# jaesung-cs/vulkan_radix_sort

Hardware: AMD Instinct MI355X
Metric: GItems/s at N=2^25 (keys & key+value); achieved HBM GB/s vs peak (higher is better)
Workload: dtype u32

## Files before the change

vulkan_radix_sort_amd/csrc/vrdx_kernels.hip:

```cpp
#include <hip/hip_runtime.h>
#include <stdint.h>

#include <type_traits>

#include "vrdx_kernels.h"
#include "vrdx_layout.h"

namespace vrdx {



#ifdef VRDX_TRACE
#define VRDX_STAMP(slot)                                      \
  do {                                                        \
    if (a.trace != nullptr && tid == 0) stamps[slot] = wall_clock64(); \
  } while (0)
#else
#define VRDX_STAMP(slot) \
  do {                   \
  } while (0)
#endif


typedef uint32_t u32x4 __attribute__((ext_vector_type(4)));
// ... 2120 lines not shown
    lo += v[k] & 0xFFFFu;
    hi += v[k] >> 16;
  }
  if (tid < 64u) {
    const uint32_t mine = tid < 2 * WORDS ? total[tid] : 0u;
    const uint32_t inclusive = WaveInclusiveScan(mine);
    if (tid < 2 * WORDS) {
      uint32_t base = inclusive - mine;
#pragma unroll
      for (uint32_t q = 0; q < 16; ++q) base += below[q];
      a.bucketBase[firstBucket + tid] = base;
      if (topWindow) a.bucketCount[firstBucket + tid] = mine;
      if (mine > a.cap) atomicOr(a.overflowWord, kMsdDeclineBucket);
    }
  }
}

template <uint32_t BITS, bool KV>
__device__ __forceinline__ void ScatterMsdBody(const MsdArgs a) {
  constexpr int THREADS = 1024, KPT = 32, WAVES = THREADS / 64;
  constexpr uint32_t TILE = kMsdTileKeys, D = 1u << BITS, ROW = D / 2u;
  static_assert(THREADS * KPT == TILE && ROW <= (uint32_t)THREADS && WAVES * ROW <= TILE, "geometry");
  extern __shared__ __attribute__((aligned(16))) uint32_t smem[];
  uint32_t* const sorted = smem;
  uint32_t* const counters = smem;
  uint32_t* const tileOffset = smem + TILE;
  uint32_t* const scanScratch = tileOffset + D;

  const int tid = threadIdx.x;
  const int lane = tid & 63;
  const int wave = tid >> 6;
  const uint32_t n = ElementCount(a.maxCount, a.countPtr);
  const uint32_t perXcd = gridDim.x / 8u;
  const uint32_t tile = (blockIdx.x % 8u) * perXcd + blockIdx.x / 8u;
  const uint32_t slots = a.tileKeys / (uint32_t)THREADS;
  const uint32_t frame = a.tileKeys;
  const uint32_t tileStart = tile * frame;
  const uint32_t decided = *a.overflowWord;
  if ((decided & kMsdDeclineMask) != 0u) {
    if (blockIdx.x == 0 && tid == 0 && a.declinedPlans != nullptr) atomicAdd(a.declinedPlans, 1u);
    return;
  }
  const uint32_t SHIFT = (decided >> kMsdShiftShift) & kMsdShiftMask;
  if (((decided >> kMsdModeShift) & kMsdModeMask) == kMsdModeIdentical) {
    if (blockIdx.x == 0 && tid == 0) *a.planWord = kMsdVerdictSorted;
    return;
  }
  const uint32_t valid = tile < a.tiles && tileStart < n ? ((n - tileStart) < frame ? (n - tileStart) : frame) : 0u;
  const uint32_t tileEnd = tileStart + valid;
  const uint32_t loadBase = tileStart + wave * (slots * 64) + lane;
  uint32_t key[KPT];
  LoadStriped<KPT, true, true>(a.keysCaller, loadBase, tileEnd, valid == frame, 0xFFFFFFFFu, key, slots);
  uint32_t prefixWord = 0, base0 = 0, base1 = 0;
  if ((uint32_t)tid < ROW && valid != 0) {
    prefixWord = a.tileCounts[(size_t)tile * ROW + tid];
    base0 = a.bucketBase[2 * tid];
    base1 = a.bucketBase[2 * tid + 1];
  }
  if (blockIdx.x == 0 && tid == 0) *a.planWord = kMsdVerdictRuns | (SHIFT << kMsdShiftShift);
  if (valid == 0) return;

  uint32_t* const myRow = counters + wave * ROW;
#pragma unroll
  for (uint32_t i = 0; i < ROW / 256u; ++i) reinterpret_cast<u32x4*>(myRow)[lane + 64 * i] = u32x4{0u, 0u, 0u, 0u};
  uint32_t rank[KPT / 2];
  RankPacked16<KPT, true>(key, SHIFT, BITS, myRow, lane, rank, slots);
  ForgetDerivedValues<KPT>(key);
  LdsBarrier();

  uint32_t column[WAVES];
  const uint32_t totals = (uint32_t)tid < ROW ? ColumnRead<ROW, WAVES>(counters, tid, column) : 0u;
  const uint32_t count0 = totals & 0xFFFFu, count1 = totals >> 16;
  const uint32_t local0 = BlockExclusiveScanAll<THREADS>(count0 + count1, scanScratch, tid);
  const uint32_t local1 = local0 + count0;
  if ((uint32_t)tid < ROW) {
    ColumnBasesFrom<ROW, WAVES>(counters, tid, local0 | (local1 << 16), column);
    tileOffset[2 * tid] = base0 + (prefixWord & 0xFFFFu) - local0;
    tileOffset[2 * tid + 1] = base1 + (prefixWord >> 16) - local1;
  }
  LdsBarrier();
  PositionsPacked16<KPT, TILE, true>(key, SHIFT, BITS, myRow, rank, slots);
  LdsBarrier();
#pragma unroll
  for (int i = 0; i < KPT; ++i) {
    if (i % 4 == 0 && (uint32_t)i >= slots) break;
    sorted[(rank[i / 2] >> (16 * (i % 2))) & 0xFFFFu] = key[i];
  }
  LdsBarrier();
  uint32_t val[KV ? KPT : 1];
  if constexpr (KV)
    LoadStriped<KPT, true, true>(a.valuesCaller, loadBase, tileEnd, valid == frame, 0u, val, slots);

  constexpr int QUADS = KPT / 4;
  constexpr int B = 4;
  uint32_t quadDigits[KV ? QUADS : 1];
  uint32_t boundaryQuad[2] = {~0u, ~0u};
  uint32_t boundaryDigits[2][2] = {{0, 0}, {0, 0}};
  if ((uint32_t)tid < ROW) {
    if (count0 != 0 && (local0 & 3u) != 0 && local0 < valid) boundaryQuad[0] = local0 & ~3u;
    if (count1 != 0 && (local1 & 3u) != 0 && local1 < valid) boundaryQuad[1] = local1 & ~3u;
  }
  if (tid == 0 && (valid & 3u) != 0) boundaryQuad[0] = valid & ~3u;
  auto scatterQuads = [&](uint32_t* out, bool keysPhase) {
#pragma unroll
    for (int j0 = 0; j0 < QUADS; j0 += B) {
      if (4u * (uint32_t)j0 * THREADS >= valid) break;
      u32x4 w4[B];
      uint32_t o[B];
      bool whole[B];
#pragma unroll
      for (int b = 0; b < B; ++b) w4[b] = *reinterpret_cast<const u32x4*>(&sorted[4u * (tid + (j0 + b) * THREADS)]);
#pragma unroll
      for (int b = 0; b < B; ++b) {
        const int j = j0 + b;
        const uint32_t p = StagingSlot<TILE>(4u * (tid + j * THREADS));
        uint32_t d0, d3;
        if (keysPhase) {
          d0 = __builtin_amdgcn_ubfe(w4[b][0], SHIFT, BITS);
          d3 = __builtin_amdgcn_ubfe(w4[b][3], SHIFT, BITS);
          if constexpr (KV) quadDigits[j] = d0 | (d3 << 16);
        } else {
          d0 = quadDigits[KV ? j : 0] & 0xFFFFu;
          d3 = quadDigits[KV ? j : 0] >> 16;
        }
        whole[b] = p + 3 < valid && d0 == d3;
        o[b] = tileOffset[d0] + p;
        asm volatile("" : "+v"(o[b]));
      }
#pragma unroll
      for (int b = 0; b < B; ++b)
        if (whole[b]) StoreQuad(out, o[b], w4[b]);
    }
#pragma unroll
    for (int s = 0; s < 2; ++s) {
      if (boundaryQuad[s] == ~0u) continue;
      const u32x4 q = *reinterpret_cast<const u32x4*>(&sorted[StagingSlot<TILE>(boundaryQuad[s])]);
      if (keysPhase) {
        boundaryDigits[s][0] = __builtin_amdgcn_ubfe(q[0], SHIFT, BITS) | (__builtin_amdgcn_ubfe(q[1], SHIFT, BITS) << 16);
        boundaryDigits[s][1] = __builtin_amdgcn_ubfe(q[2], SHIFT, BITS) | (__builtin_amdgcn_ubfe(q[3], SHIFT, BITS) << 16);
      }
#pragma unroll
      for (int c = 0; c < 4; ++c) {
        const uint32_t d = (boundaryDigits[s][c / 2] >> (16 * (c % 2))) & 0xFFFFu;
        if (boundaryQuad[s] + c < valid) StoreWord(out, tileOffset[d] + boundaryQuad[s] + c, q[c]);
      }
    }
  };
  scatterQuads(a.keysScratch, true);
  if constexpr (KV) {
    LdsBarrier();
#pragma unroll
    for (int i = 0; i < KPT; ++i) {
      if (i % 4 == 0 && (uint32_t)i >= slots) break;
      sorted[(rank[i / 2] >> (16 * (i % 2))) & 0xFFFFu] = val[i];
    }
    LdsBarrier();
    scatterQuads(a.valuesScratch, false);
  }
}

template <uint32_t BITS>
__device__ __forceinline__ void ScatterMsdPairBody(const MsdArgs a) {
  constexpr int THREADS = 1024, KPT = 32, WAVES = THREADS / 64;
  constexpr uint32_t TILE = kMsdTileKeys, D = 1u << BITS, ROW = D / 2u;
  static_assert(2 * WAVES * ROW <= TILE, "both sub-tiles' counter rows inside the staging buffer");
  extern __shared__ __attribute__((aligned(16))) uint32_t smem[];
  uint32_t* const sorted = smem;
  uint32_t* const counters = smem;
  uint32_t* const tileOffset = smem + TILE;
  uint32_t* const scanScratch = tileOffset + D;

  const int tid = threadIdx.x;
  const int lane = tid & 63;
  const int wave = tid >> 6;
  const uint32_t n = ElementCount(a.maxCount, a.countPtr);
  const uint32_t pairs = (a.tiles + 1u) / 2u;
  const uint32_t perXcd = (pairs + 7u) / 8u;
  const uint32_t pair = (blockIdx.x % 8u) * perXcd + blockIdx.x / 8u;
  const uint32_t slots = a.tileKeys / (uint32_t)THREADS;
  const uint32_t frame = a.tileKeys;
  const uint32_t decided = *a.overflowWord;
  if ((decided & kMsdDeclineMask) != 0u) {
    if (blockIdx.x == 0 && tid == 0 && a.declinedPlans != nullptr) atomicAdd(a.declinedPlans, 1u);
    return;
  }
  const uint32_t SHIFT = (decided >> kMsdShiftShift) & kMsdShiftMask;
  if (((decided >> kMsdModeShift) & kMsdModeMask) == kMsdModeIdentical) {
    if (blockIdx.x == 0 && tid == 0) *a.planWord = kMsdVerdictSorted;
    return;
  }
  const uint32_t tileA = 2u * pair;
  const uint32_t startA = tileA * frame, startB = startA + frame;
  const bool exists = blockIdx.x < 8u * perXcd && pair < pairs && startA < n;
  const uint32_t left = exists ? n - startA : 0u;
  const uint32_t validA = left < frame ? left : frame;
  const uint32_t validB = left > frame ? (left - frame < frame ? left - frame : frame) : 0u;
  const uint32_t valid = validA + validB;
  const uint32_t baseA = startA + wave * (slots * 64) + lane, baseB = baseA + frame;
  uint32_t keyA[KPT], keyB[KPT];
  LoadStriped<KPT, true, true>(a.keysCaller, baseA, startA + validA, validA == frame, 0xFFFFFFFFu, keyA, slots);
  LoadStriped<KPT, true, true>(a.keysCaller, baseB, startB + validB, validB == frame, 0xFFFFFFFFu, keyB, slots);
  uint32_t prefixWord = 0, base0 = 0, base1 = 0;
  if ((uint32_t)tid < ROW && valid != 0) {
    prefixWord = a.tileCounts[(size_t)tileA * ROW + tid];
    base0 = a.bucketBase[2 * tid];
    base1 = a.bucketBase[2 * tid + 1];
  }
  if (blockIdx.x == 0 && tid == 0) *a.planWord = kMsdVerdictRuns | (SHIFT << kMsdShiftShift);
  if (valid == 0) return;

  uint32_t* const rowA = counters + wave * ROW;
  uint32_t* const rowB = counters + (WAVES + wave) * ROW;
#pragma unroll
  for (uint32_t i = 0; i < ROW / 256u; ++i) {
    reinterpret_cast<u32x4*>(rowA)[lane + 64 * i] = u32x4{0u, 0u, 0u, 0u};
    reinterpret_cast<u32x4*>(rowB)[lane + 64 * i] = u32x4{0u, 0u, 0u, 0u};
  }
  uint32_t posA[KPT / 2], posB[KPT / 2];
  RankPacked16<KPT, true>(keyA, SHIFT, BITS, rowA, lane, posA, slots);
  ForgetDerivedValues<KPT>(keyA);
  RankPacked16<KPT, true>(keyB, SHIFT, BITS, rowB, lane, posB, slots);
  ForgetDerivedValues<KPT>(keyB);
  LdsBarrier();

  const uint32_t totals = (uint32_t)tid < ROW ? ColumnTotals<ROW, 2 * WAVES>(counters, tid) : 0u;
  const uint32_t count0 = totals & 0xFFFFu, count1 = totals >> 16;
  const uint32_t local0 = BlockExclusiveScanAll<THREADS>(count0 + count1, scanScratch, tid);
  const uint32_t local1 = local0 + count0;
  if ((uint32_t)tid < ROW) {
    ColumnBases<ROW, 2 * WAVES>(counters, tid, local0 | (local1 << 16));
    tileOffset[2 * tid] = base0 + (prefixWord & 0xFFFFu) - local0;
    tileOffset[2 * tid + 1] = base1 + (prefixWord >> 16) - local1;
  }
  LdsBarrier();
  PositionsPacked16<KPT, TILE, true, true>(keyA, SHIFT, BITS, rowA, posA, slots);
  PositionsPacked16<KPT, TILE, true, true>(keyB, SHIFT, BITS, rowB, posB, slots);
  LdsBarrier();

  constexpr int QUADS = KPT / 4;
  constexpr int B = 2;
  uint32_t boundaryQuad[2] = {~0u, ~0u};
  if ((uint32_t)tid < ROW) {
    if (count0 != 0 && (local0 & 3u) != 0 && local0 < valid) boundaryQuad[0] = local0 & ~3u;
    if (count1 != 0 && (local1 & 3u) != 0 && local1 < valid) boundaryQuad[1] = local1 & ~3u;
  }
  if (tid == 0 && (valid & 3u) != 0) boundaryQuad[0] = valid & ~3u;
#pragma unroll 1
  for (uint32_t half = 0; half < 2; ++half) {
    const uint32_t from = half * frame;
    if (from >= valid) break;
    if (half != 0) LdsBarrier();
#pragma unroll
    for (int i = 0; i < KPT; ++i) {
      if (i % 4 == 0 && (uint32_t)i >= slots) break;
      const uint32_t pa = ((posA[i / 2] >> (16 * (i % 2))) & 0xFFFFu) - from;
      const uint32_t pb = ((posB[i / 2] >> (16 * (i % 2))) & 0xFFFFu) - from;
      if (pa < frame) sorted[StagingSlot<TILE>(pa)] = keyA[i];
      if (pb < frame) sorted[StagingSlot<TILE>(pb)] = keyB[i];
    }
    LdsBarrier();
    const uint32_t here = valid - from < frame ? valid - from : frame;
#pragma unroll
    for (int j0 = 0; j0 < QUADS; j0 += B) {
      if (4u * (uint32_t)j0 * THREADS >= here) break;
      u32x4 w4[B];
      uint32_t o[B];
      bool whole[B];
#pragma unroll
      for (int b = 0; b < B; ++b) w4[b] = *reinterpret_cast<const u32x4*>(&sorted[4u * (tid + (j0 + b) * THREADS)]);
#pragma unroll
      for (int b = 0; b < B; ++b) {
        const uint32_t p = StagingSlot<TILE>(4u * (tid + (j0 + b) * THREADS));
        const uint32_t d0 = __builtin_amdgcn_ubfe(w4[b][0], SHIFT, BITS), d3 = __builtin_amdgcn_ubfe(w4[b][3], SHIFT, BITS);
        whole[b] = p + 3 < here && d0 == d3;
        o[b] = tileOffset[d0] + from + p;
        asm volatile("" : "+v"(o[b]));
      }
#pragma unroll
      for (int b = 0; b < B; ++b)
        if (whole[b]) StoreQuad(a.keysScratch, o[b], w4[b]);
    }
#pragma unroll
    for (int s = 0; s < 2; ++s) {
      const uint32_t q0 = boundaryQuad[s] - from;
      if (boundaryQuad[s] == ~0u || q0 >= frame) continue;
      const u32x4 q = *reinterpret_cast<const u32x4*>(&sorted[StagingSlot<TILE>(q0)]);
#pragma unroll
      for (int c = 0; c < 4; ++c)
        if (q0 + c < here) StoreWord(a.keysScratch, tileOffset[__builtin_amdgcn_ubfe(q[c], SHIFT, BITS)] + boundaryQuad[s] + c, q[c]);
    }
  }
}
template <uint32_t BITS, bool KV>
constexpr bool MsdScatterTakesPairs() { return !KV && BITS == 10; }
template <uint32_t BITS, bool KV>
__device__ __forceinline__ void ScatterMsdRole(const MsdArgs a) {
  if constexpr (MsdScatterTakesPairs<BITS, KV>())
    ScatterMsdPairBody<BITS>(a);
  else
    ScatterMsdBody<BITS, KV>(a);
}


template <uint32_t BITS, int KPT, bool KV, int THREADS = 1024>
__device__ __forceinline__ void BucketSort2Bucket(const MsdArgs a, const uint32_t bucket, const uint32_t below, const bool streamOut) {
  constexpr int WAVES = THREADS / 64;
  static_assert(THREADS == 1024 || THREADS == 512, "one or two words of a counter row per thread");
  constexpr uint32_t TILE = THREADS * KPT;
  constexpr uint32_t ROW = 1024;
  static_assert(32u - BITS <= 22u, "two passes of at most eleven bits");
  static_assert(TILE <= 65536 && WAVES * ROW <= TILE && KPT % 4 == 0, "packed positions; the staging buffer covers the counters");
  extern __shared__ __attribute__((aligned(16))) uint32_t smem[];
  uint32_t* const staged = smem;
  uint32_t* const counters = smem;
  uint32_t* const scanScratch = smem + TILE;

  const int tid = threadIdx.x;
  const int lane = tid & 63;
  const int wave = tid >> 6;
  const uint32_t W0 = (below + 1u) / 2u, W1 = below / 2u;
  constexpr uint32_t passes = 2u;
  const uint32_t myBase = (uint32_t)__builtin_amdgcn_readfirstlane((int)a.bucketBase[bucket]);
  const uint32_t n = (uint32_t)__builtin_amdgcn_readfirstlane((int)a.bucketCount[bucket]);
  if (n == 0) return;
  const uint32_t* const keysIn = a.keysScratch + myBase;
  uint32_t* const keysOut = a.keysCaller + myBase;
  const uint32_t* const valuesIn = KV ? a.valuesScratch + myBase : nullptr;
  uint32_t* const valuesOut = KV ? a.valuesCaller + myBase : nullptr;

  constexpr bool DYN = true;
  const uint32_t chunks = (n + 255u) / 256u;
  const uint32_t base = chunks / WAVES, extra = chunks % WAVES;
  const uint32_t w = (uint32_t)__builtin_amdgcn_readfirstlane(wave);
  const uint32_t slots = 4u * (base + (w < extra ? 1u : 0u));
  const uint32_t first = 256u * (w * base + (w < extra ? w : extra)) + lane;
  uint32_t key[KPT];
  uint32_t val[KV ? KPT : 1];
  LoadStriped<KPT, false, DYN>(keysIn, first, n, false, 0xFFFFFFFFu, key, slots);
  if constexpr (KV) LoadStriped<KPT, false, DYN>(valuesIn, first, n, false, 0u, val, slots);

  uint32_t* const myRow = counters + wave * ROW;
#pragma unroll 1
  for (uint32_t pass = 0; pass < passes; ++pass) {
    const uint32_t shift = pass == 0 ? 0u : W0;
    const uint32_t width = pass == 0 ? W0 : W1;
    const uint32_t words = width > 1u ? 1u << (width - 1u) : 1u;
#pragma unroll
    for (uint32_t i = 0; i < ROW / 256u; ++i)
      if (256u * i < words) reinterpret_cast<u32x4*>(myRow)[lane + 64 * i] = u32x4{0u, 0u, 0u, 0u};
    uint32_t rank[KPT / 2];
    RankPacked16<KPT, DYN>(key, shift, width, myRow, lane, rank, slots);
    ForgetDerivedValues<KPT>(key);
    LdsBarrier();
    uint32_t firstNow = first;
    asm volatile("" : "+v"(firstNow));
    if constexpr (THREADS == 512) {
      const bool mine = KV || 2u * (uint32_t)tid < words;
      u32x2 column[WAVES];
      const u32x2 totals = mine ? ColumnPairRead<ROW, WAVES>(counters, tid, column) : u32x2{0u, 0u};
      const uint32_t count0 = totals[0] & 0xFFFFu, count1 = totals[0] >> 16, count2 = totals[1] & 0xFFFFu;
      const uint32_t local0 = BlockExclusiveScanAll<THREADS>(count0 + count1 + count2 + (totals[1] >> 16), scanScratch + 16 * pass, tid);
      const uint32_t local2 = local0 + count0 + count1;
      if (mine)
        ColumnPairBasesFrom<ROW, WAVES>(counters, tid, u32x2{local0 | ((local0 + count0) << 16), local2 | ((local2 + count2) << 16)}, column);
    } else if constexpr (!KV) {
      const bool mine = (uint32_t)tid < words;
      uint32_t column[WAVES];
      const uint32_t totals = mine ? ColumnRead<ROW, WAVES>(counters, tid, column) : 0u;
      const uint32_t count0 = totals & 0xFFFFu;
      const uint32_t local0 = BlockExclusiveScanAll<THREADS>(count0 + (totals >> 16), scanScratch + 16 * pass, tid);
      if (mine) ColumnBasesFrom<ROW, WAVES>(counters, tid, local0 | ((local0 + count0) << 16), column);
    } else {
      const bool mine = (uint32_t)tid < words;
      const uint32_t totals = mine ? ColumnTotals<ROW, WAVES>(counters, tid) : 0u;
      const uint32_t count0 = totals & 0xFFFFu;
      const uint32_t local0 = BlockExclusiveScanAll<THREADS>(count0 + (totals >> 16), scanScratch + 16 * pass, tid);
      if (mine) ColumnBases<ROW, WAVES>(counters, tid, local0 | ((local0 + count0) << 16));
    }
    LdsBarrier();
    PositionsPacked16<KPT, TILE, DYN>(key, shift, width, myRow, rank, slots);
    LdsBarrier();
#pragma unroll
    for (int i = 0; i < KPT; ++i) {
      if (DYN && i % 4 == 0 && (uint32_t)i >= slots) break;
      staged[(rank[i / 2] >> (16 * (i % 2))) & 0xFFFFu] = key[i];
    }
    LdsBarrier();
#pragma unroll
    for (int i = 0; i < KPT; ++i) {
      if (DYN && i % 4 == 0 && (uint32_t)i >= slots) break;
      key[i] = staged[StagingSlot<TILE>(firstNow + 64 * i)];
    }
    if constexpr (KV) {
      LdsBarrier();
#pragma unroll
      for (int i = 0; i < KPT; ++i) {
        if (DYN && i % 4 == 0 && (uint32_t)i >= slots) break;
        staged[(rank[i / 2] >> (16 * (i % 2))) & 0xFFFFu] = val[i];
      }
      LdsBarrier();
#pragma unroll
      for (int i = 0; i < KPT; ++i) {
        if (DYN && i % 4 == 0 && (uint32_t)i >= slots) break;
        val[i] = staged[StagingSlot<TILE>(firstNow + 64 * i)];
      }
    }
    LdsBarrier();
  }
  if (KV ? a.maxCount > kStreamingLoadsAbove : streamOut) {
    asm volatile("; non-temporal output" ::: "memory");
#pragma unroll
    for (int i = 0; i < KPT; ++i) {
      if (DYN && i % 4 == 0 && (uint32_t)i >= slots) break;
      const uint32_t index = first + 64 * i;
      if (index < n) {
        __builtin_nontemporal_store(key[i], &keysOut[index]);
        if constexpr (KV) __builtin_nontemporal_store(val[i], &valuesOut[index]);
      }
    }
    asm volatile("" ::: "memory");
  } else {
#pragma unroll
    for (int i = 0; i < KPT; ++i) {
      if (DYN && i % 4 == 0 && (uint32_t)i >= slots) break;
      const uint32_t index = first + 64 * i;
      if (index < n) {
        keysOut[index] = key[i];
        if constexpr (KV) valuesOut[index] = val[i];
      }
    }
  }
}

template <uint32_t BITS, int KPT, bool KV, int THREADS = 1024>
__device__ __forceinline__ void BucketSort2Body(const MsdArgs a, const uint32_t workgroups) {
  const uint32_t verdict = *a.planWord;
  if ((verdict & kMsdVerdictMask) != kMsdVerdictRuns) return;
  const uint32_t below = (verdict >> kMsdShiftShift) & kMsdShiftMask;
  uint32_t streamedBuckets = 0u;
  if constexpr (!KV && THREADS == 1024 && BITS == 10)
    if (a.maxCount > kStreamingLoadsAbove) streamedBuckets = (1u << BITS) - min(a.plainTail, 1u << BITS);
#pragma unroll 1
  for (uint32_t bucket = blockIdx.x; bucket < (1u << BITS); bucket += workgroups)
    BucketSort2Bucket<BITS, KPT, KV, THREADS>(a, bucket, below, bucket < streamedBuckets);
}

template <uint32_t BITS, bool KV>
__global__ __launch_bounds__(512, 4) void bucket_sort2_half_kernel(MsdArgs a) {
  BucketSort2Body<BITS, kMsdHalfCap / 512, KV, 512>(a, gridDim.x);
}

template <uint32_t BITS, bool KV, bool DYN>
__device__ __forceinline__ void FallbackPassBody(const OnesweepArgs p) {
  if constexpr (KV)
    OnesweepBody<1024, 32, true, true, DYN>(p);
  else
    OnesweepPairBody<1024, 32, DYN>(p);
}

template <uint32_t BITS, bool KV, bool DYN>
__global__ __launch_bounds__(1024) void msd_scatter_or_pass0_kernel(MsdArgs m, OnesweepArgs p) {
  if ((*m.overflowWord & kMsdDeclineMask) == 0u) {
    ScatterMsdRole<BITS, KV>(m);
    return;
  }
  if (blockIdx.x > p.statusRows) return;
  FallbackPassBody<BITS, KV, DYN>(p);
  if (blockIdx.x == 0 && threadIdx.x == 0 && m.declinedPlans != nullptr) atomicAdd(m.declinedPlans, 1u);
}
template <uint32_t BITS, bool KV, bool DYN>
__global__ __launch_bounds__(1024) void msd_buckets_or_pass1_kernel(MsdArgs m, OnesweepArgs p) {
  const uint32_t verdict = *m.planWord & kMsdVerdictMask;
  if (verdict < kMsdVerdictRuns) {
    if (blockIdx.x > p.statusRows) return;
    FallbackPassBody<BITS, KV, DYN>(p);
    return;
  }
  const uint32_t workgroups = min(gridDim.x, (1u << BITS) / 2u);
  if (verdict == kMsdVerdictRuns && blockIdx.x < workgroups)
    BucketSort2Body<BITS, (KV ? kMsdCapKeyValue : kMsdCapKeys) / 1024, KV>(m, workgroups);
}

__device__ __forceinline__ uint32_t OrderCheckKey(uint32_t tid, uint32_t wave, uint32_t slot) {
  uint32_t x = (blockIdx.x * 1024u + tid) * 0x9E3779B9u + slot * 0x85EBCA6Bu;
  x ^= x >> 15; x *= 0x2C1B3C6Du; x ^= x >> 12; x *= 0x297A2D39u; x ^= x >> 15;
  const uint32_t mode = (blockIdx.x + wave + slot) % 6u;
  const uint32_t mask = mode == 0 ? 0u : mode == 1 ? 1u : mode == 2 ? 3u : mode == 3 ? 15u : mode == 4 ? 0x21u : 255u;
  return x & mask;
}

__global__ __launch_bounds__(1024) void lds_order_check_kernel(uint32_t* mismatches, uint32_t* sticky) {
  __shared__ uint32_t counters[2 * 16 * 256];
  const int tid = threadIdx.x, lane = tid & 63, wave = tid >> 6;
  for (int i = tid; i < 2 * 16 * 256; i += 1024) counters[i] = 0;
  __syncthreads();
  uint32_t* const histA = counters + wave * 256;
  uint32_t* const histB = counters + (16 + wave) * 256;
  uint32_t bad = 0;
  for (uint32_t round = 0; round < 8; ++round) {
    uint32_t key[8], ra[8], rb[8];
#pragma unroll
    for (int i = 0; i < 8; ++i) key[i] = OrderCheckKey(tid, wave, round * 8 + i);
    RankAtomic<8, false>(key, 0, histA, lane, ra);
    RankBallot<8>(key, 0, histB, lane, rb);
#pragma unroll
    for (int i = 0; i < 8; ++i) bad += ra[i] != rb[i];
  }
#pragma unroll 1
  for (uint32_t form = 0; form < 2; ++form) {
    uint32_t key[32], want[16];
#pragma unroll
    for (int i = 0; i < 32; ++i) key[i] = OrderCheckKey(tid, wave, 64 + 32 * form + i);
    RankBallot<32, true>(key, 0, histB, lane, want);
    if (form == 0) {
      uint32_t ra[32];
      RankAtomic<32, false>(key, 0, histA, lane, ra);
#pragma unroll
      for (int i = 0; i < 16; ++i) bad += (ra[2 * i] | (ra[2 * i + 1] << 16)) != want[i];
    } else {
      uint32_t rp[16];
      RankAtomic<32, true>(key, 0, histA, lane, rp);
#pragma unroll
      for (int i = 0; i < 16; ++i) bad += rp[i] != want[i];
    }
  }
  if (bad != 0) {
    if (mismatches != nullptr) atomicAdd(mismatches, bad);
    if (sticky != nullptr) atomicOr(sticky, 2u);
  }
}

__device__ __forceinline__ uint32_t OrderCheckDigit11(uint32_t tid, uint32_t wave, uint32_t slot) {
  uint32_t x = (blockIdx.x * 1024u + tid) * 0x9E3779B9u + slot * 0x85EBCA6Bu + 0x7F4A7C15u;
  x ^= x >> 15; x *= 0x2C1B3C6Du; x ^= x >> 12; x *= 0x297A2D39u; x ^= x >> 15;
  const uint32_t mode = (blockIdx.x + wave + slot) % 7u;
  const uint32_t mask = mode == 0 ? 0u : mode == 1 ? 1u : mode == 2 ? 3u : mode == 3 ? 15u : mode == 4 ? 0x421u : mode == 5 ? 63u : 2047u;
  return ((x & mask) + (mode == 5 ? 0x300u : 0u)) & 2047u;
}

__global__ __launch_bounds__(1024) void lds_order_check_packed_kernel(uint32_t* mismatches, uint32_t* sticky) {
  extern __shared__ __attribute__((aligned(16))) uint32_t smem[];
  const int tid = threadIdx.x, lane = tid & 63, wave = tid >> 6;
  uint32_t* const rowA = smem + wave * 1024;
  uint32_t* const rowB = smem + (16 + wave) * 1024;
  for (int i = lane; i < 1024; i += 64) rowA[i] = rowB[i] = 0;
  uint32_t bad = 0;
#pragma unroll 1
  for (uint32_t round = 0; round < 4; ++round) {
    uint32_t key[16], got[8];
#pragma unroll
    for (int i = 0; i < 16; ++i) key[i] = OrderCheckDigit11(tid, wave, round * 16 + i);
    RankPacked16<16, false>(key, 0, 11u, rowA, lane, got);
#pragma unroll
    for (int i = 0; i < 16; ++i) {
      const uint32_t d = key[i];
      uint64_t same = ~0ull;
#pragma unroll
      for (int b = 0; b < 11; ++b) {
        const bool bit = (d >> b) & 1u;
        const uint64_t ballot = __ballot(bit);
        same &= bit ? ballot : ~ballot;
      }
      const uint32_t below = LanesBelow(same);
      const uint32_t sh = (d & 1u) * 16u;
      const uint32_t prior = (__hip_atomic_load(&rowB[d >> 1], __ATOMIC_RELAXED, __HIP_MEMORY_SCOPE_WORKGROUP) >> sh) & 0xFFFFu;
      if (below == 0)
        (void)__hip_atomic_fetch_add(&rowB[d >> 1], (uint32_t)__popcll(same) << sh, __ATOMIC_RELAXED, __HIP_MEMORY_SCOPE_WORKGROUP);
      bad += ((got[i / 2] >> (16 * (i % 2))) & 0xFFFFu) != prior + below;
    }
  }
  if (bad != 0) {
    if (mismatches != nullptr) atomicAdd(mismatches, bad);
    if (sticky != nullptr) atomicOr(sticky, 2u);
  }
}

__global__ __launch_bounds__(64) void spin_kernel(unsigned long long* out, uint32_t ticks) {
  const unsigned long long t0 = wall_clock64();
  unsigned long long t = t0;
  while (t - t0 < ticks) {
    __builtin_amdgcn_s_sleep(1);
    t = wall_clock64();
  }
  if (threadIdx.x == 0) {
    out[0] = t0;
    out[1] = t;
  }
}

typedef u32x4 u32x4_a8 __attribute__((aligned(8)));

__device__ __forceinline__ uint32_t Sort64First(uint32_t n, bool* whole) {
  const uint32_t i = (blockIdx.x * kSort64Threads + threadIdx.x) * 4u;
  *whole = i + 4u <= n;
  return i;
}

struct KeyOrder64 {
  uint32_t flipHi, flipLo;
  uint32_t floatMask;
};
__device__ __forceinline__ KeyOrder64 MakeKeyOrder64(uint32_t order) {
  const uint32_t type = order & kKeyOrderTypeMask;
  const uint32_t descending = (order & kKeyOrderDescending) != 0 ? ~0u : 0u;
  return KeyOrder64{(type != kKeyOrderUint64 ? 0x80000000u : 0u) ^ descending, descending, type == kKeyOrderFloat64 ? ~0u : 0u};
}
__device__ __forceinline__ uint32_t OrderNegOfKey(const KeyOrder64& o, uint32_t hi) {
  return (uint32_t)((int32_t)hi >> 31) & o.floatMask;
}
__device__ __forceinline__ uint32_t OrderNegOfT(const KeyOrder64& o, uint32_t tHi) {
  return (uint32_t)((int32_t)(tHi ^ o.flipHi) >> 31) & o.floatMask;
}
__device__ __forceinline__ uint32_t OrderLow(const KeyOrder64& o, uint32_t lo, uint32_t neg) { return lo ^ o.flipLo ^ neg; }
__device__ __forceinline__ uint32_t OrderHigh(const KeyOrder64& o, uint32_t hi, uint32_t neg) {
  return hi ^ o.flipHi ^ (neg & 0x7FFFFFFFu);
}
__device__ __forceinline__ uint32_t OrderHighOfKey(const KeyOrder64& o, uint32_t hi) {
  return OrderHigh(o, hi, OrderNegOfKey(o, hi));
}
__device__ __forceinline__ uint32_t OrderHighOfT(const KeyOrder64& o, uint32_t tHi) {
  return OrderHigh(o, tHi, OrderNegOfT(o, tHi));
}
__device__ __forceinline__ void OrderForward(const KeyOrder64& o, uint32_t& lo, uint32_t& hi) {
  const uint32_t neg = OrderNegOfKey(o, hi);
  lo = OrderLow(o, lo, neg);
  hi = OrderHigh(o, hi, neg);
}
__device__ __forceinline__ void OrderInverse(const KeyOrder64& o, uint32_t& lo, uint32_t& hi) {
  const uint32_t neg = OrderNegOfT(o, hi);
  lo = OrderLow(o, lo, neg);
  hi = OrderHigh(o, hi, neg);
}


template <bool IOTA>
__device__ __forceinline__ void Split64(const uint64_t* __restrict__ keys, uint32_t* __restrict__ lo, uint32_t* __restrict__ other,
                                        uint32_t maxCount, const uint32_t* countPtr, uint32_t order) {
  const KeyOrder64 o = MakeKeyOrder64(order);
  const uint32_t n = ElementCount(maxCount, countPtr);
  bool whole;
  const uint32_t i = Sort64First(n, &whole);
  if (i >= n) return;
  if (whole) {
    const u32x4_a8* const pairs = reinterpret_cast<const u32x4_a8*>(keys + i);
    const u32x4 a = pairs[0], b = pairs[1];
    const u32x4 neg = u32x4{OrderNegOfKey(o, a.y), OrderNegOfKey(o, a.w), OrderNegOfKey(o, b.y), OrderNegOfKey(o, b.w)};
    *reinterpret_cast<u32x4*>(lo + i) =
        u32x4{OrderLow(o, a.x, neg.x), OrderLow(o, a.z, neg.y), OrderLow(o, b.x, neg.z), OrderLow(o, b.z, neg.w)};
    *reinterpret_cast<u32x4*>(other + i) =
        IOTA ? u32x4{i, i + 1u, i + 2u, i + 3u}
             : u32x4{OrderHigh(o, a.y, neg.x), OrderHigh(o, a.w, neg.y), OrderHigh(o, b.y, neg.z), OrderHigh(o, b.w, neg.w)};
    return;
  }
  for (uint32_t j = i; j < n; ++j) {
    const uint64_t k = keys[j];
    uint32_t l = (uint32_t)k, h = (uint32_t)(k >> 32);
    OrderForward(o, l, h);
    lo[j] = l;
    other[j] = IOTA ? j : h;
  }
}
template <bool IOTA>
__global__ __launch_bounds__(kSort64Threads) void split64_kernel(const uint64_t* __restrict__ keys, uint32_t* __restrict__ lo,
                                                                 uint32_t* __restrict__ other, uint32_t maxCount,
                                                                 const uint32_t* countPtr) {
  Split64<IOTA>(keys, lo, other, maxCount, countPtr, kKeyOrderUint64);
}
template <bool IOTA>
__global__ __launch_bounds__(kSort64Threads) void split64_ordered_kernel(const uint64_t* __restrict__ keys,
                                                                         uint32_t* __restrict__ lo,
                                                                         uint32_t* __restrict__ other, uint32_t maxCount,
                                                                         const uint32_t* countPtr, uint32_t order) {
  Split64<IOTA>(keys, lo, other, maxCount, countPtr, order);
}

__device__ __forceinline__ void Merge64(uint64_t* __restrict__ keys, const uint32_t* __restrict__ lo,
                                        const uint32_t* __restrict__ hi, uint32_t maxCount, const uint32_t* countPtr,
                                        uint32_t order) {
  const KeyOrder64 o = MakeKeyOrder64(order);
  const uint32_t n = ElementCount(maxCount, countPtr);
  bool whole;
  const uint32_t i = Sort64First(n, &whole);
  if (i >= n) return;
  if (whole) {
    const u32x4 tl = *reinterpret_cast<const u32x4*>(lo + i), th = *reinterpret_cast<const u32x4*>(hi + i);
    const u32x4 neg = u32x4{OrderNegOfT(o, th.x), OrderNegOfT(o, th.y), OrderNegOfT(o, th.z), OrderNegOfT(o, th.w)};
    const u32x4 l = u32x4{OrderLow(o, tl.x, neg.x), OrderLow(o, tl.y, neg.y), OrderLow(o, tl.z, neg.z), OrderLow(o, tl.w, neg.w)};
    const u32x4 h =
        u32x4{OrderHigh(o, th.x, neg.x), OrderHigh(o, th.y, neg.y), OrderHigh(o, th.z, neg.z), OrderHigh(o, th.w, neg.w)};
    u32x4_a8* const pairs = reinterpret_cast<u32x4_a8*>(keys + i);
    pairs[0] = u32x4{l.x, h.x, l.y, h.y};
    pairs[1] = u32x4{l.z, h.z, l.w, h.w};
    return;
  }
  for (uint32_t j = i; j < n; ++j) {
    uint32_t l = lo[j], h = hi[j];
    OrderInverse(o, l, h);
    keys[j] = (uint64_t)h << 32 | l;
  }
}
__global__ __launch_bounds__(kSort64Threads) void merge64_kernel(uint64_t* __restrict__ keys, const uint32_t* __restrict__ lo,
                                                                 const uint32_t* __restrict__ hi, uint32_t maxCount,
                                                                 const uint32_t* countPtr) {
  Merge64(keys, lo, hi, maxCount, countPtr, kKeyOrderUint64);
}
__global__ __launch_bounds__(kSort64Threads) void merge64_ordered_kernel(uint64_t* __restrict__ keys,
                                                                         const uint32_t* __restrict__ lo,
                                                                         const uint32_t* __restrict__ hi, uint32_t maxCount,
                                                                         const uint32_t* countPtr, uint32_t order) {
  Merge64(keys, lo, hi, maxCount, countPtr, order);
}

__device__ __forceinline__ void GatherHi64(const uint64_t* __restrict__ keys, const uint32_t* __restrict__ index,
                                           uint32_t* __restrict__ hi, uint32_t maxCount, const uint32_t* countPtr,
                                           uint32_t order) {
  const KeyOrder64 o = MakeKeyOrder64(order);
  const uint32_t n = ElementCount(maxCount, countPtr);
  bool whole;
  const uint32_t i = Sort64First(n, &whole);
  if (i >= n) return;
  const uint32_t* const words = reinterpret_cast<const uint32_t*>(keys);
  if (whole) {
    const u32x4 at = *reinterpret_cast<const u32x4*>(index + i);
    *reinterpret_cast<u32x4*>(hi + i) =
        u32x4{OrderHighOfKey(o, words[2ull * at.x + 1u]), OrderHighOfKey(o, words[2ull * at.y + 1u]),
              OrderHighOfKey(o, words[2ull * at.z + 1u]), OrderHighOfKey(o, words[2ull * at.w + 1u])};
    return;
  }
  for (uint32_t j = i; j < n; ++j) hi[j] = OrderHighOfKey(o, words[2ull * index[j] + 1u]);
}
__global__ __launch_bounds__(kSort64Threads) void gather_hi64_kernel(const uint64_t* __restrict__ keys,
                                                                     const uint32_t* __restrict__ index,
                                                                     uint32_t* __restrict__ hi, uint32_t maxCount,
                                                                     const uint32_t* countPtr) {
  GatherHi64(keys, index, hi, maxCount, countPtr, kKeyOrderUint64);
}
__global__ __launch_bounds__(kSort64Threads) void gather_hi64_ordered_kernel(const uint64_t* __restrict__ keys,
                                                                             const uint32_t* __restrict__ index,
                                                                             uint32_t* __restrict__ hi, uint32_t maxCount,
                                                                             const uint32_t* countPtr, uint32_t order) {
  GatherHi64(keys, index, hi, maxCount, countPtr, order);
}

__device__ __forceinline__ void Permute64(const uint64_t* __restrict__ keys, const uint32_t* __restrict__ values,
                                          const uint32_t* __restrict__ index, uint32_t* __restrict__ hiThenValues,
                                          uint64_t* __restrict__ keysOut, uint32_t maxCount, const uint32_t* countPtr,
                                          uint32_t order) {
  const KeyOrder64 o = MakeKeyOrder64(order);
  const uint32_t n = ElementCount(maxCount, countPtr);
  bool whole;
  const uint32_t i = Sort64First(n, &whole);
  if (i >= n) return;
  const uint32_t* const words = reinterpret_cast<const uint32_t*>(keys);
  if (whole) {
    const u32x4 at = *reinterpret_cast<const u32x4*>(index + i);
    const u32x4 th = *reinterpret_cast<const u32x4*>(hiThenValues + i);
    const u32x4 h = u32x4{OrderHighOfT(o, th.x), OrderHighOfT(o, th.y), OrderHighOfT(o, th.z), OrderHighOfT(o, th.w)};
    const u32x4 l = u32x4{words[2ull * at.x], words[2ull * at.y], words[2ull * at.z], words[2ull * at.w]};
    const u32x4 v = u32x4{values[at.x], values[at.y], values[at.z], values[at.w]};
    u32x4* const pairs = reinterpret_cast<u32x4*>(keysOut + i);
    pairs[0] = u32x4{l.x, h.x, l.y, h.y};
    pairs[1] = u32x4{l.z, h.z, l.w, h.w};
    *reinterpret_cast<u32x4*>(hiThenValues + i) = v;
    return;
  }
  for (uint32_t j = i; j < n; ++j) {
    const uint32_t at = index[j];
    keysOut[j] = (uint64_t)OrderHighOfT(o, hiThenValues[j]) << 32 | words[2ull * at];
    hiThenValues[j] = values[at];
  }
}
__global__ __launch_bounds__(kSort64Threads) void permute64_kernel(const uint64_t* __restrict__ keys,
                                                                   const uint32_t* __restrict__ values,
                                                                   const uint32_t* __restrict__ index,
                                                                   uint32_t* __restrict__ hiThenValues,
                                                                   uint64_t* __restrict__ keysOut, uint32_t maxCount,
                                                                   const uint32_t* countPtr) {
  Permute64(keys, values, index, hiThenValues, keysOut, maxCount, countPtr, kKeyOrderUint64);
}
__global__ __launch_bounds__(kSort64Threads) void permute64_ordered_kernel(const uint64_t* __restrict__ keys,
                                                                           const uint32_t* __restrict__ values,
                                                                           const uint32_t* __restrict__ index,
                                                                           uint32_t* __restrict__ hiThenValues,
// ... 906 lines not shown
```

Baseline: 147.8.

## Distribute MSD buckets to workgroups via atomic ticket queue instead of static stride

Bucket sorting in the combined MSD kernel now hands buckets out dynamically: each workgroup draws the next bucket index from a global atomic ticket counter and prefetches its next ticket during the last pass of the current bucket. This replaces the fixed blockIdx-strided assignment, which could leave workgroups idle when bucket sizes are skewed, and lets every launched workgroup take part instead of capping at half the bucket count. It adds one atomic per bucket and an extra LDS word past the tile, and it depends on the ticket counter (a.tickets+1) being reset before each sort. The half-size kernel keeps static striding.

```diff
diff --git a/vulkan_radix_sort_amd/csrc/vrdx_kernels.hip b/vulkan_radix_sort_amd/csrc/vrdx_kernels.hip
--- a/vulkan_radix_sort_amd/csrc/vrdx_kernels.hip
+++ b/vulkan_radix_sort_amd/csrc/vrdx_kernels.hip
@@ -2446,8 +2446,9 @@
 }
 
 
-template <uint32_t BITS, int KPT, bool KV, int THREADS = 1024>
-__device__ __forceinline__ void BucketSort2Bucket(const MsdArgs a, const uint32_t bucket, const uint32_t below, const bool streamOut) {
+template <uint32_t BITS, int KPT, bool KV, int THREADS = 1024, bool DRAW = true>
+__device__ __forceinline__ void BucketSort2Bucket(const MsdArgs a, const uint32_t bucket, const uint32_t below, const bool streamOut,
+                                                  uint32_t* const ticketWord, uint32_t* const nextDrawn) {
   constexpr int WAVES = THREADS / 64;
   static_assert(THREADS == 1024 || THREADS == 512, "one or two words of a counter row per thread");
   constexpr uint32_t TILE = THREADS * KPT;
@@ -2466,7 +2467,13 @@
   constexpr uint32_t passes = 2u;
   const uint32_t myBase = (uint32_t)__builtin_amdgcn_readfirstlane((int)a.bucketBase[bucket]);
   const uint32_t n = (uint32_t)__builtin_amdgcn_readfirstlane((int)a.bucketCount[bucket]);
-  if (n == 0) return;
+  if (n == 0) {
+    if constexpr (DRAW) {
+      if (tid == 0) *nextDrawn = atomicAdd(ticketWord, 1u);
+      LdsBarrier();
+    }
+    return;
+  }
   const uint32_t* const keysIn = a.keysScratch + myBase;
   uint32_t* const keysOut = a.keysCaller + myBase;
   const uint32_t* const valuesIn = KV ? a.valuesScratch + myBase : nullptr;
@@ -2524,6 +2531,12 @@
     LdsBarrier();
     PositionsPacked16<KPT, TILE, DYN>(key, shift, width, myRow, rank, slots);
     LdsBarrier();
+    uint32_t drawn = 0;
+    if (DRAW && pass + 1u == passes && tid == 0) {
+      uint32_t none = 0;
+      asm volatile("" : "+v"(none));
+      drawn = atomicAdd(ticketWord + none, 1u);
+    }
 #pragma unroll
     for (int i = 0; i < KPT; ++i) {
       if (DYN && i % 4 == 0 && (uint32_t)i >= slots) break;
@@ -2549,6 +2562,7 @@
         val[i] = staged[StagingSlot<TILE>(firstNow + 64 * i)];
       }
     }
+    if (DRAW && pass + 1u == passes && tid == 0) *nextDrawn = drawn;
     LdsBarrier();
   }
   if (KV ? a.maxCount > kStreamingLoadsAbove : streamOut) {
@@ -2576,22 +2590,36 @@
   }
 }
 
-template <uint32_t BITS, int KPT, bool KV, int THREADS = 1024>
-__device__ __forceinline__ void BucketSort2Body(const MsdArgs a, const uint32_t workgroups) {
+template <uint32_t BITS, int KPT, bool KV>
+__device__ __forceinline__ void BucketSort2Body(const MsdArgs a) {
+  constexpr int THREADS = 1024;
   const uint32_t verdict = *a.planWord;
   if ((verdict & kMsdVerdictMask) != kMsdVerdictRuns) return;
   const uint32_t below = (verdict >> kMsdShiftShift) & kMsdShiftMask;
   uint32_t streamedBuckets = 0u;
-  if constexpr (!KV && THREADS == 1024 && BITS == 10)
+  if constexpr (!KV && BITS == 10)
     if (a.maxCount > kStreamingLoadsAbove) streamedBuckets = (1u << BITS) - min(a.plainTail, 1u << BITS);
+  extern __shared__ __attribute__((aligned(16))) uint32_t smem[];
+  uint32_t* const drawn = smem + THREADS * KPT;
+  uint32_t* const ticketWord = a.tickets + 1;
+  if (threadIdx.x == 0) drawn[0] = atomicAdd(ticketWord, 1u);
+  LdsBarrier();
 #pragma unroll 1
-  for (uint32_t bucket = blockIdx.x; bucket < (1u << BITS); bucket += workgroups)
-    BucketSort2Bucket<BITS, KPT, KV, THREADS>(a, bucket, below, bucket < streamedBuckets);
+  for (uint32_t turn = 0;; turn ^= 1u) {
+    const uint32_t bucket = (uint32_t)__builtin_amdgcn_readfirstlane((int)drawn[turn]);
+    if (bucket >= (1u << BITS)) return;
+    BucketSort2Bucket<BITS, KPT, KV, THREADS>(a, bucket, below, bucket < streamedBuckets, ticketWord, drawn + (turn ^ 1u));
+  }
 }
 
 template <uint32_t BITS, bool KV>
 __global__ __launch_bounds__(512, 4) void bucket_sort2_half_kernel(MsdArgs a) {
-  BucketSort2Body<BITS, kMsdHalfCap / 512, KV, 512>(a, gridDim.x);
+  const uint32_t verdict = *a.planWord;
+  if ((verdict & kMsdVerdictMask) != kMsdVerdictRuns) return;
+  const uint32_t below = (verdict >> kMsdShiftShift) & kMsdShiftMask;
+#pragma unroll 1
+  for (uint32_t bucket = blockIdx.x; bucket < (1u << BITS); bucket += gridDim.x)
+    BucketSort2Bucket<BITS, kMsdHalfCap / 512, KV, 512, false>(a, bucket, below, false, nullptr, nullptr);
 }
 
 template <uint32_t BITS, bool KV, bool DYN>
@@ -2620,9 +2648,7 @@
     FallbackPassBody<BITS, KV, DYN>(p);
     return;
   }
-  const uint32_t workgroups = min(gridDim.x, (1u << BITS) / 2u);
-  if (verdict == kMsdVerdictRuns && blockIdx.x < workgroups)
-    BucketSort2Body<BITS, (KV ? kMsdCapKeyValue : kMsdCapKeys) / 1024, KV>(m, workgroups);
+  if (verdict == kMsdVerdictRuns) BucketSort2Body<BITS, (KV ? kMsdCapKeyValue : kMsdCapKeys) / 1024, KV>(m);
 }
 
 __device__ __forceinline__ uint32_t OrderCheckKey(uint32_t tid, uint32_t wave, uint32_t slot) {
```

Result: faster. 151.5 (median of 6 runs) (+2.5%).
